# koadman/mauveAligner

Hardware: AMD Instinct MI355X
Metric: aligned Mbp/s (seed+extend+DP) (higher is better)
Workload: dtype u32; 1 GPU; C3: 5 x 5000000 bp synthetic genomes, ~3% divergence, ~50 inversions, seed weight 15, recursive anchoring + gapped DP on; genomes_per_gpu=5, genome_length=5000000, seed_weight=15, parallelism=independent genome sets per GPU (no data-path collective), extend_lcbs=1, max_extension_iters=4

## Files before the change

### mauvealigner_amd/csrc/radix_sort.hip

```cpp
#include "radix_sort.hpp"
#include <algorithm>
#include <cstdlib>

template <typename KeyT>
__global__ void __launch_bounds__(RS_THREADS) rs_hist(const KeyT *__restrict__ keys, uint32_t n, int shift,
                                                      uint32_t *__restrict__ hist, uint32_t nblk)
{
    __shared__ uint32_t h[256];
    h[threadIdx.x] = 0;
    __syncthreads();
    const uint32_t base = blockIdx.x * RS_TILE;
    if (base + RS_TILE <= n) {
        constexpr int KPV = 16 / (int)sizeof(KeyT);
        struct alignas(16) Vec { KeyT k[KPV]; };
        const Vec *src = reinterpret_cast<const Vec *>(keys + base);
#pragma unroll
        for (int i = 0; i < RS_ITEMS / KPV; i++) {
            const Vec q = src[i * RS_THREADS + threadIdx.x];
#pragma unroll
            for (int j = 0; j < KPV; j++) atomicAdd(&h[(uint32_t)(q.k[j] >> shift) & 255u], 1u);
        }
    } else {
#pragma unroll
        for (int i = 0; i < RS_ITEMS; i++) {
// ... 37 lines not shown
    for (uint32_t i0 = lo; i0 < hi; i0 += 512) {
        uint32_t v[8];
#pragma unroll
        for (int q = 0; q < 8; q++) { const uint32_t idx = i0 + q * 64 + lane; v[q] = idx < hi ? row[idx] : 0u; }
#pragma unroll
        for (int q = 0; q < 8; q++) {
            const uint32_t idx = i0 + q * 64 + lane;
            const uint32_t inc = wave_incl_sum_u32(v[q]);
            if (idx < hi) row[idx] = run + inc - v[q];
            run += (uint32_t)__builtin_amdgcn_readlane((int32_t)inc, 63);
        }
    }
    if (threadIdx.x == 0) totals[blockIdx.x] = total;
}

template <typename KeyT, bool RAW = false, typename ValT = uint32_t>
__global__ void __launch_bounds__(RS_THREADS) rs_scatter(const KeyT *__restrict__ keys_in,
                                                         const ValT *__restrict__ vals_in,
                                                         KeyT *__restrict__ keys_out,
                                                         ValT *__restrict__ vals_out, uint32_t n, int shift,
                                                         const uint32_t *__restrict__ hist,
                                                         const uint32_t *__restrict__ totals, uint32_t nblk)
{
    __shared__ KeyT s_keys[RS_TILE];
    __shared__ ValT s_vals[RS_TILE];
    __shared__ uint32_t wcount[RS_WAVES][256];
    __shared__ uint32_t gbase[256];
    __shared__ uint32_t tstart[256];
    __shared__ uint32_t scan[256];

    const int tid = threadIdx.x;
// ... 2 lines not shown

    for (int w = 0; w < RS_WAVES; w++) wcount[w][tid] = 0;
    if (RAW) {
        const uint32_t *row = hist + (size_t)tid * nblk;
        uint32_t tot = 0, before = 0;
        for (uint32_t t = 0; t < nblk; t++) { const uint32_t c = row[t]; tot += c; before += t < blockIdx.x ? c : 0u; }
        uint32_t dummy;
        gbase[tid] = block_excl_scan(tot, &dummy, scan) + before;
    } else {
        uint32_t dummy;
        const uint32_t tot = totals[tid];
        gbase[tid] = block_excl_scan(tot, &dummy, scan) + hist[(size_t)tid * nblk + blockIdx.x];
    }
    __syncthreads();
    if (tile_n == RS_TILE)
        rs_scatter_tile<KeyT, RS_ITEMS, true, ValT>(keys_in, vals_in, keys_out, vals_out, tile_base, tile_n, shift, s_keys, s_vals, wcount, gbase, tstart, scan);
    else
        rs_scatter_tile<KeyT, RS_ITEMS, false, ValT>(keys_in, vals_in, keys_out, vals_out, tile_base, tile_n, shift, s_keys, s_vals, wcount, gbase, tstart, scan);
}

static bool small_sort_on() { static const bool v = [] { const char *e = getenv("MAUVE_SMALL_SORT"); return !(e && e[0] == '0'); }(); return v; }

template <typename KeyT, typename ValT>
int sort_pairs(mauve_ctx *ctx, uint32_t n, int key_bits, KeyT **keys_io, ValT **vals_io, KeyT *keys_alt, ValT *vals_alt, bool have_hist0,
               int timer_id, int shift_lo)
{
    const int k_hist = timer_id >= 0 ? timer_id : MAUVE_K_SORT_HIST, k_scan = timer_id >= 0 ? timer_id : MAUVE_K_SORT_SCAN,
              k_scat = timer_id >= 0 ? timer_id : MAUVE_K_SORT_SCATTER;
    if (small_sort_on() && !have_hist0 && n >= 1 && n <= SS_CAP) {
        HIPCHK(ctx, ctx->hist.ensure(ss_ws_words(n) * sizeof(uint32_t)));
        small_sort<KeyT>(ctx->stream, n, key_bits, shift_lo, keys_io, vals_io, keys_alt, vals_alt, ctx->hist.as<uint32_t>(),
                         [&](bool scatter, auto &&launch) { KernelTimer t(ctx, scatter ? k_scat : k_hist, n); launch(); });
        HIPCHK(ctx, hipGetLastError());
        return MAUVE_OK;
    }
    uint32_t nblk = (n + RS_TILE - 1) / RS_TILE;
    HIPCHK(ctx, ctx->hist.ensure((size_t)nblk * 256 * sizeof(uint32_t)));
    HIPCHK(ctx, ctx->totals.ensure(256 * sizeof(uint32_t)));
    KeyT *kin = *keys_io, *kout = keys_alt; ValT *vin = *vals_io, *vout = vals_alt;
    for (int shift = shift_lo; shift < key_bits; shift += 8) {
        if (!(shift == shift_lo && have_hist0)) { KernelTimer t(ctx, k_hist, n);
          hipLaunchKernelGGL(rs_hist<KeyT>, dim3(nblk), dim3(RS_THREADS), 0, ctx->stream, kin, n, shift,
                             ctx->hist.as<uint32_t>(), nblk); }
        if (nblk <= 64) {
            KernelTimer t(ctx, k_scat, n);
            hipLaunchKernelGGL((rs_scatter<KeyT, true, ValT>), dim3(nblk), dim3(RS_THREADS), 0, ctx->stream, kin, vin, kout, vout, n,
                               shift, ctx->hist.as<uint32_t>(), ctx->totals.as<uint32_t>(), nblk);
            std::swap(kin, kout); std::swap(vin, vout);
            continue;
        }
        { KernelTimer t(ctx, k_scan, n);
          hipLaunchKernelGGL(rs_rowscan, dim3(256), dim3(256), 0, ctx->stream, ctx->hist.as<uint32_t>(), nblk,
                             ctx->totals.as<uint32_t>()); }
        { KernelTimer t(ctx, k_scat, n);
          hipLaunchKernelGGL((rs_scatter<KeyT, false, ValT>), dim3(nblk), dim3(RS_THREADS), 0, ctx->stream, kin, vin, kout, vout, n,
                             shift, ctx->hist.as<uint32_t>(), ctx->totals.as<uint32_t>(), nblk); }
        std::swap(kin, kout); std::swap(vin, vout);
    }
    HIPCHK(ctx, hipGetLastError());
    *keys_io = kin; *vals_io = vin;
    return MAUVE_OK;
}
RS_SORT_PAIRS(uint32_t, uint32_t);
RS_SORT_PAIRS(uint32_t, uint64_t);
RS_SORT_PAIRS(uint64_t, uint32_t);
RS_SORT_PAIRS(uint64_t, uint64_t);

int sort_pairs_u32(mauve_ctx *ctx, uint32_t n, int key_bits, uint32_t **keys_io, uint32_t **vals_io, uint32_t *keys_alt, uint32_t *vals_alt,
                   int timer_id)
{
    return sort_pairs<uint32_t>(ctx, n, key_bits, keys_io, vals_io, keys_alt, vals_alt, false, timer_id);
// ... 30 lines not shown
```

### mauvealigner_amd/csrc/radix_sort.hpp

```cpp
#pragma once
#include "common.hpp"
#include "small_sort.hpp"

constexpr int RS_ITEMS = 16;
constexpr int RS_TILE = RS_THREADS * RS_ITEMS;

template <typename KeyT, typename ValT = uint32_t>
int sort_pairs(mauve_ctx *ctx, uint32_t n, int key_bits, KeyT **keys_io, ValT **vals_io, KeyT *keys_alt, ValT *vals_alt, bool have_hist0,
               int timer_id = -1, int shift_lo = 0);
#define RS_SORT_PAIRS(KeyT, ValT) template int sort_pairs<KeyT, ValT>(mauve_ctx *, uint32_t, int, KeyT **, ValT **, KeyT *, ValT *, bool, int, int)
extern RS_SORT_PAIRS(uint32_t, uint32_t);
extern RS_SORT_PAIRS(uint32_t, uint64_t);
extern RS_SORT_PAIRS(uint64_t, uint32_t);
extern RS_SORT_PAIRS(uint64_t, uint64_t);
```

### mauvealigner_amd/csrc/seed_pass.hip

```cpp
#include "common.hpp"
#include "dev_scan.hpp"
#include "radix_sort.hpp"
#include "seed_dev.hpp"
#include <algorithm>
#include <cstring>
#include <cstdlib>
#include <type_traits>

__device__ __forceinline__ uint32_t seg_of(const uint32_t *__restrict__ segs, uint32_t nseg, uint32_t p)
{
    uint32_t lo = 0, hi = nseg;
    while (hi - lo > 1) { uint32_t mid = (lo + hi) >> 1; if (segs[mid] <= p) lo = mid; else hi = mid; }
    return lo;
}
__device__ __forceinline__ bool window_segment(const uint32_t *__restrict__ seg, uint32_t nseg, int g, uint32_t p, int span, uint32_t *id)
{
    const uint32_t *sg = seg + (size_t)g * (nseg + 1);
    const uint32_t k = *id = seg_of(sg, nseg, p);
    return p + span <= sg[k + 1];
}

template <typename KeyT, bool SEG, typename ValT = uint32_t>
__global__ void __launch_bounds__(256) seed_extract(const uint64_t *__restrict__ packed, GenomeTab tab,
                                                    SeedShape sh, int g, KeyT *__restrict__ keys,
// ... 8 lines not shown
        if (SEG) {
            uint32_t k;
            key = window_segment(seg, nseg, g, p, sh.span, &k) ? (((uint64_t)k << (2 * sh.weight)) | key) : ~0ULL;
        }
        keys[out_base + p] = (KeyT)key;
        vals[out_base + p] = win_make<ValT>(tab.gpos_off[g] + p, m.strand);
    }
}

template <typename KeyT, bool SEG, bool NARROW, typename ValT = uint32_t>
__global__ void __launch_bounds__(256) seed_extract_all(const uint64_t *__restrict__ packed, GenomeTab tab, SeedShape sh,
                                                        KeyT *__restrict__ keys, ValT *__restrict__ vals, uint32_t P,
                                                        const uint32_t *__restrict__ seg, uint32_t nseg,
                                                        uint32_t *__restrict__ hist, uint32_t nblk,
                                                        const uint64_t *__restrict__ vmask, int hist_shift,
                                                        const uint64_t *__restrict__ cmask)
{
    __shared__ uint32_t h[256];
    h[threadIdx.x] = 0;
    __syncthreads();
    const uint32_t base = blockIdx.x * 4096u;
#pragma unroll 2
    for (int i = 0; i < 4; i++) {
        const uint32_t gp0 = base + i * 1024 + threadIdx.x * 4;
        if (gp0 >= P) break;
        const int g0 = genome_of(gp0, tab);
        const bool together = gp0 + 3 < P && gp0 + 3 < tab.gpos_off[g0 + 1];
        uint64_t key[4]; uint32_t sf[4];
        if (together) {
            const uint32_t p0 = gp0 - tab.gpos_off[g0];
            const uint64_t *G = packed + tab.word_off[g0];
            const uint32_t q = p0 >> 5; const int r0 = (p0 & 31) * 2;
            const uint64_t w0 = G[q], w1 = G[q + 1], w2 = G[q + 2], w3 = NARROW ? 0ULL : G[q + 3];
#pragma unroll
// ... 17 lines not shown
        }
        if (SEG || vmask || cmask) {
#pragma unroll
            for (int j = 0; j < 4; j++) {
                const uint32_t gp = gp0 + j;
                if (gp >= P) continue;
                const int g = together ? g0 : genome_of(gp, tab);
                const uint32_t p = gp - tab.gpos_off[g];
                if (SEG) {
                    uint32_t k;
                    key[j] = window_segment(seg, nseg, g, p, sh.span, &k) ? (((uint64_t)k << (2 * sh.weight)) | key[j]) : ~0ULL;
                }
                if ((vmask || cmask) && window_blocked(vmask ? vmask + tab.mask_off[g] : nullptr, cmask ? cmask + tab.mask_off[g] : nullptr, p, sh.span)) key[j] = ~0ULL;
            }
        }
        if (gp0 + 3 < P) {
            if (sizeof(KeyT) == 4) *reinterpret_cast<uint4 *>(keys + gp0) = make_uint4((uint32_t)key[0], (uint32_t)key[1], (uint32_t)key[2], (uint32_t)key[3]);
            else {
                reinterpret_cast<ulonglong2 *>(keys + gp0)[0] = make_ulonglong2(key[0], key[1]);
                reinterpret_cast<ulonglong2 *>(keys + gp0)[1] = make_ulonglong2(key[2], key[3]);
            }
            if constexpr (sizeof(ValT) == 4)
                *reinterpret_cast<uint4 *>(vals + gp0) = make_uint4(gp0 | (sf[0] << 31), (gp0 + 1) | (sf[1] << 31), (gp0 + 2) | (sf[2] << 31), (gp0 + 3) | (sf[3] << 31));
            else {
                reinterpret_cast<ulonglong2 *>(vals + gp0)[0] = make_ulonglong2(win_make<ValT>(gp0, sf[0]), win_make<ValT>(gp0 + 1, sf[1]));
                reinterpret_cast<ulonglong2 *>(vals + gp0)[1] = make_ulonglong2(win_make<ValT>(gp0 + 2, sf[2]), win_make<ValT>(gp0 + 3, sf[3]));
            }
#pragma unroll
            for (int j = 0; j < 4; j++) atomicAdd(&h[(uint32_t)((KeyT)key[j] >> hist_shift) & 255u], 1u);
        } else {
            for (int j = 0; j < 4 && gp0 + j < P; j++) {
                keys[gp0 + j] = (KeyT)key[j]; vals[gp0 + j] = win_make<ValT>(gp0 + j, sf[j]);
                atomicAdd(&h[(uint32_t)((KeyT)key[j] >> hist_shift) & 255u], 1u);
            }
        }
    }
    __syncthreads();
    hist[threadIdx.x * nblk + blockIdx.x] = h[threadIdx.x];
}

__device__ __forceinline__ bool window_valid(uint32_t gp, uint32_t P, const GenomeTab &tab, int span, const uint64_t *__restrict__ vmask,
                                             const uint64_t *__restrict__ cmask)
{
    if (gp >= P) return false;
    const int g = genome_of(gp, tab);
    return !window_blocked(vmask ? vmask + tab.mask_off[g] : nullptr, cmask ? cmask + tab.mask_off[g] : nullptr, gp - tab.gpos_off[g], span);
}

__global__ void __launch_bounds__(256) valid_count(GenomeTab tab, int span, uint32_t P, const uint64_t *__restrict__ vmask,
                                                   uint32_t *__restrict__ tile_cnt, const uint64_t *__restrict__ cmask)
{
    __shared__ uint32_t lds[8];
    const uint32_t first = blockIdx.x * 4096u + threadIdx.x * 16u;
// ... 213 lines not shown
        const uint32_t m = finder_components(mode, once, multi, want_mask);
        if (!(m & gbit[r])) continue;
        mm[r] = m;
        if ((m & (0u - m)) == gbit[r]) skey[slot[r]] = sizeof(ValT) == 4 ? (KeyT)v[r] : (KeyT)win_idx(v[r]);
    }
    __syncthreads();
#pragma unroll
    for (int r = 0; r < HJ_ROWS; r++) {
        if (!mm[r]) continue;
        const uint32_t ap = sizeof(ValT) == 4 ? (uint32_t)skey[slot[r]] & 0x7fffffffu : (uint32_t)skey[slot[r]];
        if (ap >= P) { atomicAdd(&ovf_cnt[1], 1u); continue; }
        const int g = __ffs(gbit[r]) - 1;
        tpos[(size_t)ap * tab.nseq + g] = hit_word(v[r], tab.gpos_off[g]);
        if ((mm[r] & (0u - mm[r])) == gbit[r]) tmask[ap] = mm[r];
    }
}

constexpr int TJ_SLOTS = 16384;
constexpr int TJ_MAX = 9216;
constexpr int TJ_ROWS = TJ_MAX / 1024;
template <bool LOCAL = false>
__global__ void __launch_bounds__(1024) tiny_join(const uint64_t *__restrict__ packed, GenomeTab tab, SeedShape sh, uint32_t P,
                                                  const uint64_t *__restrict__ vmask, const uint64_t *__restrict__ cmask, int mode, uint32_t want_mask,
                                                  uint32_t *__restrict__ tmask, uint32_t *__restrict__ tpos, uint32_t *__restrict__ err_cnt,
                                                  const uint32_t *__restrict__ seg, uint32_t nseg, uint32_t *__restrict__ counters, uint32_t clr_lo, uint32_t clr_hi)
{
    extern __shared__ uint32_t tj_lds[];
    uint32_t *skey = tj_lds, *som = tj_lds + TJ_SLOTS;
    constexpr uint32_t EMPTY = 0xffffffffu;
    const int tid = threadIdx.x;
// ... 533 lines not shown
    tab->gpos_off[gs.nseq] = (uint32_t)tot;
    for (int g = gs.nseq + 1; g <= MAUVE_MAX_SEQ; g++) tab->gpos_off[g] = 0xffffffffu;
    *total_windows = tot;
    return MAUVE_OK;
}

struct FinderPass { uint32_t consider, want; int rule; };

struct SeedPlan {
    bool seg;
    bool hash_path;
    bool tiny;
    bool compact;
    bool has_invalid;
    bool use_summary;
    int segbits;
    int full_bits;
    int low_bits(uint32_t entries) const
    {
        if (!hash_path) return 0;
        int G = 0;
        while (G < full_bits && ((uint64_t)entries >> G) > 512) G += 8;
        if (seg) G = std::max(G, (segbits + 7) / 8 * 8);
        return full_bits - std::min(G, full_bits);
    }
};

static int seed_plan(mauve_ctx *ctx, const SeedShape &sh, const GenomeTab &tab, const SeedRequest &rq, uint32_t n, bool masked, bool seg,
                     int key_type_bits, SeedPlan *pl, std::vector<FinderPass> *passes)
{
    pl->seg = seg;
    pl->hash_path = !rq.hits && rq.mode != MAUVE_MODE_PAIRWISE && !rq.out_keys && !rq.enumerate && rq.only_seq < 0 && !(masked && seg);
    pl->segbits = 0;
    if (seg) while (pl->segbits < 32 && (1ull << pl->segbits) <= (uint64_t)rq.nseg) pl->segbits++;
    if (seg && 2 * sh.weight + pl->segbits > 64) { ctx->err = "recursive anchoring: segment id and mer do not fit 64 bits"; return MAUVE_ERR_LIMIT; }
    pl->full_bits = seg ? 2 * sh.weight + pl->segbits : ((masked && rq.only_seq >= 0) ? key_type_bits : 2 * sh.weight);
    pl->tiny = pl->hash_path && !no_tiny() && n <= (uint32_t)TJ_MAX && tab.nseq <= 16 && 2 * sh.weight + pl->segbits <= 32;
    pl->compact = !rq.hits && !pl->tiny && rq.only_seq < 0 && masked && !seg;
    pl->has_invalid = masked && !pl->compact;
    const int N = tab.nseq;
    if (rq.mode == MAUVE_MODE_PAIRWISE) {
        int pi = 0;
        for (int i = 0; i < N; i++) for (int j = i + 1; j < N; j++, pi++)
            if (!ctx->pair_sums_only || !ctx->shard_on || pi % ctx->shard_world == ctx->shard_rank)
                passes->push_back({(1u << i) | (1u << j), (1u << i) | (1u << j), MAUVE_MODE_MEM});
    } else passes->push_back({0xffffffffu, (uint32_t)rq.mask, rq.mode});
    pl->use_summary = rq.mode == MAUVE_MODE_PAIRWISE && !seg && !rq.hits && (passes->size() > 1 || (ctx->pair_sums_only && ctx->shard_on && !passes->empty()));
    return MAUVE_OK;
}

struct SeedState {
    mauve_ctx *ctx; const GenomeSet &gs; const SeedShape &sh; const GenomeTab &tab; const SeedRequest &rq;
    uint32_t P;
    const uint64_t *packed, *vmask, *cmask;
    SeedPlan pl;
    std::vector<FinderPass> passes;
    uint32_t ns = 0;
    int L = 0;
    uint32_t *tmask = nullptr, *tpos = nullptr;
    uint32_t cand_cap = 0;
    uint32_t cand_total = 0;
    bool records_on_host = false;
    double trace_t0 = 0;
};
template <typename KeyT, typename ValT>
struct SeedPass : SeedState {
    KeyT *keys = nullptr; ValT *vals = nullptr;
    bool have_hist0 = false;
    SeedPass(const SeedState &s) : SeedState(s) {}
};

template <typename KeyT, typename ValT>
static int ensure_sort_buffers(mauve_ctx *ctx, uint32_t n)
{
    HIPCHK(ctx, ctx->keysA.ensure((size_t)n * sizeof(KeyT)));
    HIPCHK(ctx, ctx->keysB.ensure((size_t)n * sizeof(KeyT)));
    HIPCHK(ctx, ctx->valsA.ensure((size_t)n * sizeof(ValT)));
    HIPCHK(ctx, ctx->valsB.ensure((size_t)n * sizeof(ValT)));
    return MAUVE_OK;
}

template <typename F>
static void launch_narrow_or_not(const SeedShape &sh, F &&launch)
{
    if (seed_narrow(sh)) launch(std::true_type{});
    else launch(std::false_type{});
}

template <typename KeyT, bool SEG, typename ValT>
static int extract_all(mauve_ctx *ctx, const GenomeSet &gs, const SeedShape &sh, const GenomeTab &tab, uint32_t n, const uint32_t *seg, uint32_t nseg,
                       int hshift, KeyT *keys, ValT *vals)
{
    const uint32_t nblk = (n + RS_TILE - 1) / RS_TILE;
    HIPCHK(ctx, ctx->hist.ensure((size_t)nblk * 256 * sizeof(uint32_t)));
    const uint64_t *packed = gs.buf->as<uint64_t>();
    const uint64_t *vmask = gs.vmask ? gs.vmask->as<uint64_t>() : nullptr;
    const uint64_t *cmask = gs.cmask ? gs.cmask->as<uint64_t>() : nullptr;
    KernelTimer t(ctx, MAUVE_K_EXTRACT, n);
    launch_narrow_or_not(sh, [&](auto narrow) {
        hipLaunchKernelGGL((seed_extract_all<KeyT, SEG, decltype(narrow)::value, ValT>), dim3(nblk), dim3(256), 0, ctx->stream, packed, tab, sh, keys,
                           vals, n, seg, nseg, ctx->hist.as<uint32_t>(), nblk, vmask, hshift, cmask);
    });
    return MAUVE_OK;
}

template <typename KeyT, bool SEG, typename ValT>
static int extract(SeedPass<KeyT, ValT> &ps)
{
    mauve_ctx *ctx = ps.ctx; const SeedRequest &rq = ps.rq; const uint32_t n = ps.P;
    if (int rc = ensure_sort_buffers<KeyT, ValT>(ctx, n)) return rc;
    HIPCHK(ctx, ctx->counters.ensure(64));
    KeyT *keys = ps.keys = ctx->keysA.as<KeyT>(); ValT *vals = ps.vals = ctx->valsA.as<ValT>();
    if (rq.hits) ps.ns = 1;
    else if (ps.pl.tiny) ps.ns = n;
    else if (ps.pl.compact) {
        const uint32_t nblk = (n + 4095) / 4096;
// ... 1 lines not shown
        uint32_t *tile_cnt = ctx->hist.as<uint32_t>();
        {
            KernelTimer t(ctx, MAUVE_K_EXTRACT, n);
            hipLaunchKernelGGL(valid_count, dim3(nblk), dim3(256), 0, ctx->stream, ps.tab, ps.sh.span, n, ps.vmask, tile_cnt, ps.cmask);
            hipLaunchKernelGGL(tile_scan, dim3(1), dim3(256), 0, ctx->stream, tile_cnt, nblk, ctx->counters.as<uint32_t>());
            launch_narrow_or_not(ps.sh, [&](auto narrow) {
                hipLaunchKernelGGL((seed_extract_compact<KeyT, decltype(narrow)::value, ValT>), dim3(nblk), dim3(256), 0, ctx->stream, ps.packed, ps.tab, ps.sh,
                                   keys, vals, n, ps.vmask, tile_cnt, ps.cmask);
            });
        }
        HIPCHK(ctx, hipGetLastError());
        const uint32_t *cw;
        if (int rc = seed_counters(ctx, 16, &cw)) return rc;
        ps.ns = cw[0];
    } else if (rq.only_seq < 0) {
        if (int rc = extract_all<KeyT, SEG, ValT>(ctx, ps.gs, ps.sh, ps.tab, n, rq.seg, rq.nseg, ps.pl.low_bits(n), keys, vals)) return rc;
        ps.ns = n; ps.have_hist0 = true;
    } else {
        const int g = rq.only_seq;
        uint32_t nw = ps.tab.nwin[g];
        if (nw) {
            uint32_t blocks = std::min<uint32_t>((nw + 255) / 256, 256 * 16);
            KernelTimer t(ctx, MAUVE_K_EXTRACT, nw);
            hipLaunchKernelGGL((seed_extract<KeyT, SEG, ValT>), dim3(blocks), dim3(256), 0, ctx->stream, ps.packed, ps.tab, ps.sh, g, keys,
                               vals, 0u, rq.seg, rq.nseg);
            ps.ns = nw;
        }
    }
    HIPCHK(ctx, hipGetLastError());
    seed_trace(ctx, "extract", ps.trace_t0);
    return MAUVE_OK;
}
// ... 49 lines not shown
    out_keys->resize(sorted_n);
    for (uint32_t i = 0; i < sorted_n; i++) (*out_keys)[i] = (uint64_t)hk[i];
    if (WIDEV) {
        const uint32_t g0 = ps.tab.gpos_off[ps.rq.only_seq];
        for (uint32_t i = 0; i < sorted_n; i++) (*out_vals)[i] = ((uint32_t)hv[i] - g0) | ((uint32_t)((uint64_t)hv[i] >> 63) << 31);
    }
    return MAUVE_OK;
}

static bool cand_overflow(SeedState &st, uint32_t nc)
{
    if (nc > st.cand_cap) st.ctx->err = "seed pass: " + std::to_string(nc) + " candidates for a list of " + std::to_string(st.cand_cap);
    return nc > st.cand_cap;
}

template <bool SEG>
static int launch_runs(SeedState &st)
{
    mauve_ctx *ctx = st.ctx; const uint32_t P = st.P;
    { KernelTimer t(ctx, MAUVE_K_RUNS, P);
      hipLaunchKernelGGL((mum_runs<SEG>), dim3((P + RUNS_TILE - 1) / RUNS_TILE), dim3(256), 0, ctx->stream, st.tab,
                         st.sh.span, st.tmask, st.tpos, P, st.rq.extend ? 0 : 1, ctx->cand.as<uint32_t>(), ctx->counters.as<uint32_t>(), st.rq.seg,
                         st.rq.nseg, st.cand_cap, 0u); }
    HIPCHK(ctx, hipGetLastError());
    return MAUVE_OK;
}

template <bool SEG, bool WIDEV>
static int launch_extend(SeedState &st, uint32_t blocks, uint32_t ncand, int32_t *o_len, int32_t *o_start, const uint32_t *ncand_dev = nullptr,
                         uint32_t *counters_out = nullptr)
{
    mauve_ctx *ctx = st.ctx;
    KernelTimer t(ctx, MAUVE_K_EXTEND, ncand);
    hipLaunchKernelGGL((mum_extend<SEG, WIDEV>), dim3(blocks), dim3(256), 0, ctx->stream, st.packed, st.tab, st.sh, st.tmask, st.tpos, st.P,
                       ctx->cand.as<uint32_t>(), ncand, st.rq.extend, o_len, o_start, st.rq.seg, st.rq.nseg, st.vmask, st.cmask, ncand_dev, counters_out);
    HIPCHK(ctx, hipGetLastError());
#ifdef MAUVE_EXT_STATS
    if (seed_trace_on()) {
// ... 80 lines not shown
    return MAUVE_OK;
}

static_assert(TJ_MAX / 2 + 1 <= 8192, "a tiny pass's candidate list: extension launched for its capacity");
template <bool SEG, bool WIDEV>
static int tiny_pass(SeedState &st, const FinderPass &fp)
{
    mauve_ctx *ctx = st.ctx; const uint32_t P = st.P, cand_cap = st.cand_cap; const int N = st.tab.nseq;
    static const bool tj_attr = hipFuncSetAttribute(reinterpret_cast<const void *>(tiny_join<WIDEV>), hipFuncAttributeMaxDynamicSharedMemorySize, TJ_SLOTS * 8) == hipSuccess;
    if (!tj_attr) { ctx->err = "tiny_join: cannot reserve its LDS"; return MAUVE_ERR_HIP; }
    { KernelTimer t(ctx, MAUVE_K_JOIN, P);
      hipLaunchKernelGGL(tiny_join<WIDEV>, dim3(1), dim3(1024), TJ_SLOTS * 8, ctx->stream, st.packed, st.tab, st.sh, P, st.vmask, st.cmask, fp.rule, fp.want, st.tmask, st.tpos,
                         ctx->counters.as<uint32_t>() + 9, SEG ? st.rq.seg : (const uint32_t *)nullptr, st.rq.nseg, ctx->counters.as<uint32_t>(), 0u, P); }
    HIPCHK(ctx, hipGetLastError());
    seed_trace(ctx, "join", st.trace_t0);
    if (int rc = launch_runs<SEG>(st)) return rc;
    if (ctx->shadow) { std::function<void()> f; f.swap(ctx->shadow); f(); }
    const size_t lbytes = ((size_t)cand_cap * 4 + 63) & ~(size_t)63, sbytes = (size_t)cand_cap * 4 * N;
    HIPCHK(ctx, ctx->pin_seed.ensure(64 + lbytes + sbytes));
    char *pin = ctx->pin_seed.as<char>();
    const bool host_out = cand_cap < canon_device_min();
    if (!host_out) { HIPCHK(ctx, ctx->mlen.ensure((size_t)cand_cap * 4 + 4)); HIPCHK(ctx, ctx->mstart.ensure((size_t)cand_cap * 4 * N + 4)); }
    int32_t *o_len = host_out ? reinterpret_cast<int32_t *>(pin + 64) : ctx->mlen.as<int32_t>();
    int32_t *o_st = host_out ? reinterpret_cast<int32_t *>(pin + 64 + lbytes) : ctx->mstart.as<int32_t>();
    if (int rc = launch_extend<SEG, WIDEV>(st, std::min<uint32_t>((cand_cap + 3) / 4, 512), cand_cap, o_len, o_st, ctx->counters.as<uint32_t>() + 1,
                                           reinterpret_cast<uint32_t *>(pin))) return rc;
    if (!host_out) {
        HIPCHK(ctx, hipMemcpyAsync(pin + 64, ctx->mlen.p, (size_t)cand_cap * 4, hipMemcpyDeviceToHost, ctx->stream));
        HIPCHK(ctx, hipMemcpyAsync(pin + 64 + lbytes, ctx->mstart.p, sbytes, hipMemcpyDeviceToHost, ctx->stream));
    }
    HIPCHK(ctx, hipStreamSynchronize(ctx->stream));
// ... 35 lines not shown
    }
    if (tot_sl) {
        HIPCHK(ctx, ctx->join_bound.ensure((2 * nsl + 1) * 4));
        HIPCHK(ctx, ctx->pin_seed.ensure(64 + (2 * nsl + 1) * 4));
        uint32_t *hp = reinterpret_cast<uint32_t *>(ctx->pin_seed.as<char>() + 64);
        memcpy(hp, sl_lo.data(), nsl * 4); memcpy(hp + nsl, sl_pre.data(), (nsl + 1) * 4);
        HIPCHK(ctx, hipMemcpyAsync(ctx->join_bound.p, hp, (2 * nsl + 1) * 4, hipMemcpyHostToDevice, ctx->stream));
        KernelTimer t(ctx, MAUVE_K_JOIN, (uint32_t)tot_sl);
        hipLaunchKernelGGL((mum_join_slices<KeyT, SEG, ValT>), dim3((uint32_t)((tot_sl + 255) / 256)), dim3(256), 0, ctx->stream, (const KeyT *)keys, (const ValT *)vals,
                           ctx->join_bound.as<uint32_t>(), ctx->join_bound.as<uint32_t>() + nsl, (uint32_t)nsl, ps.tab, fp.rule, fp.want,
                           fp.consider, ps.tmask, ps.tpos, (int)ps.pl.has_invalid);
        HIPCHK(ctx, hipStreamSynchronize(ctx->stream));
    }
    HIPCHK(ctx, hipGetLastError());
    HIPCHK(ctx, hipMemsetAsync(ctx->counters.p, 0, 64, ctx->stream));
    if (int rc = launch_runs<SEG>(ps)) return rc;
    const uint32_t *cw;
    if (int rc = seed_counters(ctx, 16, &cw)) return rc;
    *nc = cw[1];
    if (seed_trace_on()) fprintf(stderr, "[trace]   join_hash handed back %u range(s)\n", novf);
    return MAUVE_OK;
}

template <typename KeyT, bool SEG, typename ValT>
static int finder_pass(SeedPass<KeyT, ValT> &ps, const FinderPass &fp)
{
    constexpr bool WIDEV = sizeof(ValT) == 8;
    mauve_ctx *ctx = ps.ctx; const uint32_t P = ps.P, ns = ps.ns; const int N = ps.tab.nseq;
    const HostHits *hh = ps.rq.hits;
    HIPCHK(ctx, hipMemsetAsync(ps.tmask, 0, (size_t)P * 4, ctx->stream));
    HIPCHK(ctx, hipMemsetAsync(ctx->counters.p, 0, 64, ctx->stream));
    if (hh) {
        HIPCHK(ctx, ctx->run_sum.ensure((size_t)hh->n * (N + 1) * 4 + 64));
        HIPCHK(ctx, hipMemcpyAsync(ctx->run_sum.p, hh->rec, (size_t)hh->n * (N + 1) * 4, hipMemcpyHostToDevice, ctx->stream));
        if (hh->n) hipLaunchKernelGGL(hits_scatter<WIDEV>, dim3((hh->n + 255) / 256), dim3(256), 0, ctx->stream, ctx->run_sum.as<uint32_t>(), hh->n, N, P, ps.tmask, ps.tpos, ps.tab);
        HIPCHK(ctx, hipStreamSynchronize(ctx->stream));
    } else if (ps.pl.hash_path) {
        const uint32_t nchunk = (ns + HJ_T - 1) / HJ_T;
        HIPCHK(ctx, ctx->join_ovf.ensure((2 + 2 * (size_t)HJ_OVF_CAP) * 4));
        KernelTimer t(ctx, MAUVE_K_JOIN, ns);
        HIPCHK(ctx, ctx->join_bound.ensure(((size_t)nchunk + 2) * 4));
        hipLaunchKernelGGL((join_bounds<KeyT>), dim3((nchunk + 1 + 3) / 4), dim3(256), 0, ctx->stream, ps.keys, ns, ps.L, nchunk,
                           ctx->join_bound.as<uint32_t>());
#define JH_LAUNCH(W) hipLaunchKernelGGL((join_hash<KeyT, W, ValT>), dim3(nchunk), dim3(256), 0, ctx->stream, ps.keys, ps.vals, ns, \
                                           ctx->join_bound.as<uint32_t>(), ps.tab, fp.rule, fp.want, ps.tmask, ps.tpos, ctx->counters.as<uint32_t>() + 8, ctx->join_ovf.as<uint32_t>(), P)
        if (N > 16) JH_LAUNCH(true);
        else JH_LAUNCH(false);
#undef JH_LAUNCH
    } else
    { KernelTimer t(ctx, MAUVE_K_JOIN, ns);
      hipLaunchKernelGGL((mum_join<KeyT, SEG, ValT>), dim3((ns + 255) / 256), dim3(256), 0, ctx->stream, ps.keys, ps.vals, ns, ps.tab, fp.rule,
                         fp.want, fp.consider, ps.tmask, ps.tpos, P, (int)ps.pl.has_invalid); }
    HIPCHK(ctx, hipGetLastError());
    seed_trace(ctx, "join", ps.trace_t0);
    if (int rc = launch_runs<SEG>(ps)) return rc;
    if (ctx->shadow) { std::function<void()> f; f.swap(ctx->shadow); f(); }
    const uint32_t *cw;
    if (int rc = seed_counters(ctx, 48, &cw)) return rc;
    uint32_t nc = cw[1];
    const uint32_t novf = ps.pl.hash_path ? cw[8] : 0u;
    if (ps.pl.hash_path && cw[9]) { ctx->err = "join_hash: anchor out of range (internal error)"; return MAUVE_ERR_HIP; }
    if (novf) if (int rc = join_overflow_slices<KeyT, SEG, ValT>(ps, fp, novf, &nc)) return rc;
    if (cand_overflow(ps, nc)) return MAUVE_ERR_LIMIT;
    seed_trace(ctx, "runs", ps.trace_t0);
    if (seed_trace_on()) fprintf(stderr, "[trace]   %u candidates of %u windows\n", nc, P);
    if (nc == 0) return MAUVE_OK;
    constexpr int EXT_BLOCKS_PER_CU = 12;
    return extend_candidates<SEG, WIDEV>(ps, nc, (uint32_t)(ctx->cus * EXT_BLOCKS_PER_CU));
}

template <typename KeyT, bool SEG, typename ValT>
static int seedpass_stages(const SeedState &st0)
{
    constexpr bool WIDEV = sizeof(ValT) == 8;
    SeedPass<KeyT, ValT> ps(st0);
    mauve_ctx *ctx = ps.ctx; const SeedRequest &rq = ps.rq; const uint32_t P = ps.P; const int N = ps.tab.nseq;
    if (seed_trace_on()) fprintf(stderr, "[trace] seed pass: %u windows, %d-bit keys, %s window index (%d-bit values)\n", P, (int)sizeof(KeyT) * 8,
                                  WIDEV ? "wide" : "narrow", (int)sizeof(ValT) * 8);
    if (int rc = seed_plan(ctx, ps.sh, ps.tab, rq, P, ps.vmask || ps.cmask, SEG, (int)sizeof(KeyT) * 8, &ps.pl, &ps.passes)) return rc;
    if (int rc = extract<KeyT, SEG, ValT>(ps)) return rc;
    if (ps.ns == 0) { if (rq.n_matches) *rq.n_matches = 0; return MAUVE_OK; }
    ps.L = ps.pl.low_bits(ps.ns);
    if (!rq.hits && !ps.pl.tiny)
        if (int rc = sort_pairs<KeyT, ValT>(ctx, ps.ns, ps.pl.full_bits, &ps.keys, &ps.vals, ctx->keysB.as<KeyT>(), ctx->valsB.as<ValT>(), ps.have_hist0, -1, ps.L)) return rc;
    seed_trace(ctx, "sort", ps.trace_t0);
    if (rq.enumerate) return export_enumerator(ps);
    if (rq.out_keys) return export_sorted_list(ps);

    HIPCHK(ctx, ctx->posmask.ensure((size_t)P * 4));
    HIPCHK(ctx, ctx->hit_pos.ensure((size_t)P * 4 * N));
    ps.tmask = ctx->posmask.as<uint32_t>(); ps.tpos = ctx->hit_pos.as<uint32_t>();
    ps.cand_cap = P / 2 + 1;
    HIPCHK(ctx, ctx->cand.ensure((size_t)ps.cand_cap * 4));
    if (list_cap_env()) ps.cand_cap = std::min(ps.cand_cap, list_cap_env());
    ctx->sdh.hl.clear(); ctx->sdh.hs.clear();
    if (ps.pl.tiny) {
        if (int rc = tiny_pass<SEG, WIDEV>(ps, ps.passes[0])) return rc;
    } else if (ps.pl.use_summary) {
        if (int rc = pairwise_passes(ps)) return rc;
// ... 194 lines not shown
```

### mauvealigner_amd/csrc/small_sort.hpp

```cpp
#pragma once
#include <hip/hip_runtime.h>
#include <cstdint>

constexpr int RS_THREADS = 256;
constexpr int RS_WAVES = RS_THREADS / 64;

__device__ __forceinline__ uint32_t block_excl_scan(uint32_t v, uint32_t *total, uint32_t *lds )
{
    const int lane = threadIdx.x & 63, wave = threadIdx.x >> 6;
    uint32_t inc = v;
#pragma unroll
    for (int o = 1; o < 64; o <<= 1) { uint32_t t = __shfl_up(inc, o); if (lane >= o) inc += t; }
    if (lane == 63) lds[wave] = inc;
    __syncthreads();
    uint32_t wbase = 0, tot = 0;
#pragma unroll
    for (int w = 0; w < 4; w++) { uint32_t c = lds[w]; if (w < wave) wbase += c; tot += c; }
    __syncthreads();
    *total = tot;
    return wbase + inc - v;
}

template <typename KeyT, int ITEMS, bool FULL, typename ValT = uint32_t>
__device__ __forceinline__ void rs_scatter_tile(const KeyT *__restrict__ keys_in, const ValT *__restrict__ vals_in,
                                                KeyT *__restrict__ keys_out, ValT *__restrict__ vals_out,
                                                uint32_t tile_base, uint32_t tile_n, int shift, KeyT *s_keys, ValT *s_vals,
                                                uint32_t (*wcount)[256], const uint32_t *gbase, uint32_t *tstart, uint32_t *scan,
                                                uint32_t *__restrict__ hnext = nullptr, int tile_log2 = 0, int hbits = 0)
{
    const int tid = threadIdx.x, lane = tid & 63, wave = tid >> 6;
    KeyT k[ITEMS]; ValT v[ITEMS]; uint32_t rank[ITEMS];
    const uint32_t wbase = wave * (64 * ITEMS);
#pragma unroll
    for (int i = 0; i < ITEMS; i++) {
        const uint32_t li = wbase + i * 64 + lane;
        const bool ok = FULL || li < tile_n;
        k[i] = ok ? keys_in[tile_base + li] : (KeyT)0;
        v[i] = ok ? vals_in[tile_base + li] : (ValT)0;
    }
    uint32_t *wc = wcount[wave];
#pragma unroll
    for (int i = 0; i < ITEMS; i++) {
        const uint32_t li = wbase + i * 64 + lane;
        const bool ok = FULL || li < tile_n;
        const uint32_t d = (uint32_t)(k[i] >> shift) & 255u;
        uint32_t plo, phi;
        if (FULL) { plo = 0xffffffffu; phi = 0xffffffffu; }
        else { const uint64_t a = __ballot(ok); plo = (uint32_t)a; phi = (uint32_t)(a >> 32); }
#pragma unroll
        for (int b = 0; b < 8; b++) {
            const uint64_t m = FULL ? __ballot((d >> b) & 1) : __ballot(ok && ((d >> b) & 1));
            const uint32_t sb = (uint32_t)((int32_t)(d << (31 - b)) >> 31);
            plo &= ~((uint32_t)m ^ sb); phi &= ~((uint32_t)(m >> 32) ^ sb);
// ... 174 lines not shown
```

Before: 10110 Mbp/s.

## Pack strand bits into a bitmap and synthesize sort values in first scatter

Seed extraction no longer writes a full per-window value array. It now writes a compact bitmap of strand flags per tile, and the first radix scatter pass reconstructs each value from the element index plus the bitmap bit. The finder pass replaces the full-array memset of the mask with a custom clear kernel limited to the window range the pass anchors on, and restricts mum_runs to that range. This cuts global memory writes and reads of the value stream and the clear cost, but adds template variants and a dependency on the first pass being tiled.

```diff
diff --git a/mauvealigner_amd/csrc/radix_sort.hip b/mauvealigner_amd/csrc/radix_sort.hip
--- a/mauvealigner_amd/csrc/radix_sort.hip
+++ b/mauvealigner_amd/csrc/radix_sort.hip
@@ -75,7 +75,7 @@
     if (threadIdx.x == 0) totals[blockIdx.x] = total;
 }
 
-template <typename KeyT, bool RAW = false, typename ValT = uint32_t>
+template <typename KeyT, bool RAW = false, typename ValT = uint32_t, bool IOTA = false>
 __global__ void __launch_bounds__(RS_THREADS) rs_scatter(const KeyT *__restrict__ keys_in,
                                                          const ValT *__restrict__ vals_in,
                                                          KeyT *__restrict__ keys_out,
@@ -108,19 +108,22 @@
     }
     __syncthreads();
     if (tile_n == RS_TILE)
-        rs_scatter_tile<KeyT, RS_ITEMS, true, ValT>(keys_in, vals_in, keys_out, vals_out, tile_base, tile_n, shift, s_keys, s_vals, wcount, gbase, tstart, scan);
+        rs_scatter_tile<KeyT, RS_ITEMS, true, ValT, IOTA>(keys_in, vals_in, keys_out, vals_out, tile_base, tile_n, shift, s_keys, s_vals, wcount, gbase, tstart, scan,
+                                                          nullptr, 0, 0, reinterpret_cast<const uint64_t *>(vals_in));
     else
-        rs_scatter_tile<KeyT, RS_ITEMS, false, ValT>(keys_in, vals_in, keys_out, vals_out, tile_base, tile_n, shift, s_keys, s_vals, wcount, gbase, tstart, scan);
+        rs_scatter_tile<KeyT, RS_ITEMS, false, ValT, IOTA>(keys_in, vals_in, keys_out, vals_out, tile_base, tile_n, shift, s_keys, s_vals, wcount, gbase, tstart, scan,
+                                                           nullptr, 0, 0, reinterpret_cast<const uint64_t *>(vals_in));
 }
 
 static bool small_sort_on() { static const bool v = [] { const char *e = getenv("MAUVE_SMALL_SORT"); return !(e && e[0] == '0'); }(); return v; }
 
 template <typename KeyT, typename ValT>
 int sort_pairs(mauve_ctx *ctx, uint32_t n, int key_bits, KeyT **keys_io, ValT **vals_io, KeyT *keys_alt, ValT *vals_alt, bool have_hist0,
-               int timer_id, int shift_lo)
+               int timer_id, int shift_lo, bool iota)
 {
     const int k_hist = timer_id >= 0 ? timer_id : MAUVE_K_SORT_HIST, k_scan = timer_id >= 0 ? timer_id : MAUVE_K_SORT_SCAN,
               k_scat = timer_id >= 0 ? timer_id : MAUVE_K_SORT_SCATTER;
+    if (iota && !(have_hist0 && shift_lo < key_bits)) { ctx->err = "sort_pairs: values from the strand bitmap need a first tiled pass"; return MAUVE_ERR_ARG; }
     if (small_sort_on() && !have_hist0 && n >= 1 && n <= SS_CAP) {
         HIPCHK(ctx, ctx->hist.ensure(ss_ws_words(n) * sizeof(uint32_t)));
         small_sort<KeyT>(ctx->stream, n, key_bits, shift_lo, keys_io, vals_io, keys_alt, vals_alt, ctx->hist.as<uint32_t>(),
@@ -136,10 +139,11 @@
         if (!(shift == shift_lo && have_hist0)) { KernelTimer t(ctx, k_hist, n);
           hipLaunchKernelGGL(rs_hist<KeyT>, dim3(nblk), dim3(RS_THREADS), 0, ctx->stream, kin, n, shift,
                              ctx->hist.as<uint32_t>(), nblk); }
+        const bool first_iota = iota && shift == shift_lo;
         if (nblk <= 64) {
             KernelTimer t(ctx, k_scat, n);
-            hipLaunchKernelGGL((rs_scatter<KeyT, true, ValT>), dim3(nblk), dim3(RS_THREADS), 0, ctx->stream, kin, vin, kout, vout, n,
-                               shift, ctx->hist.as<uint32_t>(), ctx->totals.as<uint32_t>(), nblk);
+            hipLaunchKernelGGL((first_iota ? rs_scatter<KeyT, true, ValT, true> : rs_scatter<KeyT, true, ValT, false>), dim3(nblk), dim3(RS_THREADS), 0, ctx->stream,
+                               kin, vin, kout, vout, n, shift, ctx->hist.as<uint32_t>(), ctx->totals.as<uint32_t>(), nblk);
             std::swap(kin, kout); std::swap(vin, vout);
             continue;
         }
@@ -147,8 +151,8 @@
           hipLaunchKernelGGL(rs_rowscan, dim3(256), dim3(256), 0, ctx->stream, ctx->hist.as<uint32_t>(), nblk,
                              ctx->totals.as<uint32_t>()); }
         { KernelTimer t(ctx, k_scat, n);
-          hipLaunchKernelGGL((rs_scatter<KeyT, false, ValT>), dim3(nblk), dim3(RS_THREADS), 0, ctx->stream, kin, vin, kout, vout, n,
-                             shift, ctx->hist.as<uint32_t>(), ctx->totals.as<uint32_t>(), nblk); }
+          hipLaunchKernelGGL((first_iota ? rs_scatter<KeyT, false, ValT, true> : rs_scatter<KeyT, false, ValT, false>), dim3(nblk), dim3(RS_THREADS), 0, ctx->stream,
+                             kin, vin, kout, vout, n, shift, ctx->hist.as<uint32_t>(), ctx->totals.as<uint32_t>(), nblk); }
         std::swap(kin, kout); std::swap(vin, vout);
     }
     HIPCHK(ctx, hipGetLastError());
diff --git a/mauvealigner_amd/csrc/radix_sort.hpp b/mauvealigner_amd/csrc/radix_sort.hpp
--- a/mauvealigner_amd/csrc/radix_sort.hpp
+++ b/mauvealigner_amd/csrc/radix_sort.hpp
@@ -7,8 +7,8 @@
 
 template <typename KeyT, typename ValT = uint32_t>
 int sort_pairs(mauve_ctx *ctx, uint32_t n, int key_bits, KeyT **keys_io, ValT **vals_io, KeyT *keys_alt, ValT *vals_alt, bool have_hist0,
-               int timer_id = -1, int shift_lo = 0);
-#define RS_SORT_PAIRS(KeyT, ValT) template int sort_pairs<KeyT, ValT>(mauve_ctx *, uint32_t, int, KeyT **, ValT **, KeyT *, ValT *, bool, int, int)
+               int timer_id = -1, int shift_lo = 0, bool iota = false);
+#define RS_SORT_PAIRS(KeyT, ValT) template int sort_pairs<KeyT, ValT>(mauve_ctx *, uint32_t, int, KeyT **, ValT **, KeyT *, ValT *, bool, int, int, bool)
 extern RS_SORT_PAIRS(uint32_t, uint32_t);
 extern RS_SORT_PAIRS(uint32_t, uint64_t);
 extern RS_SORT_PAIRS(uint64_t, uint32_t);
diff --git a/mauvealigner_amd/csrc/seed_pass.hip b/mauvealigner_amd/csrc/seed_pass.hip
--- a/mauvealigner_amd/csrc/seed_pass.hip
+++ b/mauvealigner_amd/csrc/seed_pass.hip
@@ -46,10 +46,12 @@
                                                         const uint32_t *__restrict__ seg, uint32_t nseg,
                                                         uint32_t *__restrict__ hist, uint32_t nblk,
                                                         const uint64_t *__restrict__ vmask, int hist_shift,
-                                                        const uint64_t *__restrict__ cmask)
+                                                        const uint64_t *__restrict__ cmask, uint32_t *__restrict__ sbits)
 {
     __shared__ uint32_t h[256];
+    __shared__ uint32_t sb[4096 / 32];
     h[threadIdx.x] = 0;
+    if (threadIdx.x < 4096 / 32) sb[threadIdx.x] = 0;
     __syncthreads();
     const uint32_t base = blockIdx.x * 4096u;
 #pragma unroll 2
@@ -97,13 +99,15 @@
                 if ((vmask || cmask) && window_blocked(vmask ? vmask + tab.mask_off[g] : nullptr, cmask ? cmask + tab.mask_off[g] : nullptr, p, sh.span)) key[j] = ~0ULL;
             }
         }
+        if (sbits) atomicOr(&sb[(gp0 - base) >> 5], (sf[0] | sf[1] << 1 | sf[2] << 2 | sf[3] << 3) << ((gp0 - base) & 31u));
         if (gp0 + 3 < P) {
             if (sizeof(KeyT) == 4) *reinterpret_cast<uint4 *>(keys + gp0) = make_uint4((uint32_t)key[0], (uint32_t)key[1], (uint32_t)key[2], (uint32_t)key[3]);
             else {
                 reinterpret_cast<ulonglong2 *>(keys + gp0)[0] = make_ulonglong2(key[0], key[1]);
                 reinterpret_cast<ulonglong2 *>(keys + gp0)[1] = make_ulonglong2(key[2], key[3]);
             }
-            if constexpr (sizeof(ValT) == 4)
+            if (sbits) {}
+            else if constexpr (sizeof(ValT) == 4)
                 *reinterpret_cast<uint4 *>(vals + gp0) = make_uint4(gp0 | (sf[0] << 31), (gp0 + 1) | (sf[1] << 31), (gp0 + 2) | (sf[2] << 31), (gp0 + 3) | (sf[3] << 31));
             else {
                 reinterpret_cast<ulonglong2 *>(vals + gp0)[0] = make_ulonglong2(win_make<ValT>(gp0, sf[0]), win_make<ValT>(gp0 + 1, sf[1]));
@@ -113,13 +117,15 @@
             for (int j = 0; j < 4; j++) atomicAdd(&h[(uint32_t)((KeyT)key[j] >> hist_shift) & 255u], 1u);
         } else {
             for (int j = 0; j < 4 && gp0 + j < P; j++) {
-                keys[gp0 + j] = (KeyT)key[j]; vals[gp0 + j] = win_make<ValT>(gp0 + j, sf[j]);
+                keys[gp0 + j] = (KeyT)key[j];
+                if (!sbits) vals[gp0 + j] = win_make<ValT>(gp0 + j, sf[j]);
                 atomicAdd(&h[(uint32_t)((KeyT)key[j] >> hist_shift) & 255u], 1u);
             }
         }
     }
     __syncthreads();
     hist[threadIdx.x * nblk + blockIdx.x] = h[threadIdx.x];
+    if (sbits && threadIdx.x < 4096 / 32) sbits[(size_t)blockIdx.x * (4096 / 32) + threadIdx.x] = sb[threadIdx.x];
 }
 
 __device__ __forceinline__ bool window_valid(uint32_t gp, uint32_t P, const GenomeTab &tab, int span, const uint64_t *__restrict__ vmask,
@@ -363,6 +369,17 @@
         tpos[(size_t)ap * tab.nseq + g] = hit_word(v[r], tab.gpos_off[g]);
         if ((mm[r] & (0u - mm[r])) == gbit[r]) tmask[ap] = mm[r];
     }
+}
+
+__global__ void __launch_bounds__(256) pass_clear(uint32_t *__restrict__ t, uint32_t n, uint32_t *__restrict__ counters)
+{
+    if (blockIdx.x == 0 && threadIdx.x < 16) counters[threadIdx.x] = 0;
+    const uint32_t head = (uint32_t)((reinterpret_cast<uintptr_t>(t) >> 2) & 3u);
+    const uint64_t w = ((uint64_t)blockIdx.x * 256u + threadIdx.x) * 4u;
+    if (w >= (uint64_t)head + n) return;
+    uint32_t *line = t - head + w;
+    if (w >= head && w + 4 <= (uint64_t)head + n) *reinterpret_cast<uint4 *>(line) = make_uint4(0u, 0u, 0u, 0u);
+    else for (uint32_t j = 0; j < 4; j++) if (w + j >= head && w + j < (uint64_t)head + n) line[j] = 0;
 }
 
 constexpr int TJ_SLOTS = 16384;
@@ -926,6 +943,7 @@
     bool compact;
     bool has_invalid;
     bool use_summary;
+    bool strand_bitmap;
     int segbits;
     int full_bits;
     int low_bits(uint32_t entries) const
@@ -950,6 +968,7 @@
     pl->tiny = pl->hash_path && !no_tiny() && n <= (uint32_t)TJ_MAX && tab.nseq <= 16 && 2 * sh.weight + pl->segbits <= 32;
     pl->compact = !rq.hits && !pl->tiny && rq.only_seq < 0 && masked && !seg;
     pl->has_invalid = masked && !pl->compact;
+    pl->strand_bitmap = !rq.hits && !pl->tiny && !pl->compact && rq.only_seq < 0 && pl->low_bits(n) < pl->full_bits;
     const int N = tab.nseq;
     if (rq.mode == MAUVE_MODE_PAIRWISE) {
         int pi = 0;
@@ -979,6 +998,7 @@
 struct SeedPass : SeedState {
     KeyT *keys = nullptr; ValT *vals = nullptr;
     bool have_hist0 = false;
+    bool iota = false;
     SeedPass(const SeedState &s) : SeedState(s) {}
 };
 
@@ -1001,7 +1021,7 @@
 
 template <typename KeyT, bool SEG, typename ValT>
 static int extract_all(mauve_ctx *ctx, const GenomeSet &gs, const SeedShape &sh, const GenomeTab &tab, uint32_t n, const uint32_t *seg, uint32_t nseg,
-                       int hshift, KeyT *keys, ValT *vals)
+                       int hshift, KeyT *keys, ValT *vals, bool bitmap = false)
 {
     const uint32_t nblk = (n + RS_TILE - 1) / RS_TILE;
     HIPCHK(ctx, ctx->hist.ensure((size_t)nblk * 256 * sizeof(uint32_t)));
@@ -1011,7 +1031,7 @@
     KernelTimer t(ctx, MAUVE_K_EXTRACT, n);
     launch_narrow_or_not(sh, [&](auto narrow) {
         hipLaunchKernelGGL((seed_extract_all<KeyT, SEG, decltype(narrow)::value, ValT>), dim3(nblk), dim3(256), 0, ctx->stream, packed, tab, sh, keys,
-                           vals, n, seg, nseg, ctx->hist.as<uint32_t>(), nblk, vmask, hshift, cmask);
+                           vals, n, seg, nseg, ctx->hist.as<uint32_t>(), nblk, vmask, hshift, cmask, bitmap ? reinterpret_cast<uint32_t *>(vals) : nullptr);
     });
     return MAUVE_OK;
 }
@@ -1043,8 +1063,10 @@
         if (int rc = seed_counters(ctx, 16, &cw)) return rc;
         ps.ns = cw[0];
     } else if (rq.only_seq < 0) {
-        if (int rc = extract_all<KeyT, SEG, ValT>(ctx, ps.gs, ps.sh, ps.tab, n, rq.seg, rq.nseg, ps.pl.low_bits(n), keys, vals)) return rc;
-        ps.ns = n; ps.have_hist0 = true;
+        if (ps.pl.strand_bitmap) HIPCHK(ctx, ctx->valsA.ensure(std::max((size_t)n * sizeof(ValT), (size_t)((n + RS_TILE - 1) / RS_TILE) * (RS_TILE / 8))));
+        vals = ps.vals = ctx->valsA.as<ValT>();
+        if (int rc = extract_all<KeyT, SEG, ValT>(ctx, ps.gs, ps.sh, ps.tab, n, rq.seg, rq.nseg, ps.pl.low_bits(n), keys, vals, ps.pl.strand_bitmap)) return rc;
+        ps.ns = n; ps.have_hist0 = true; ps.iota = ps.pl.strand_bitmap;
     } else {
         const int g = rq.only_seq;
         uint32_t nw = ps.tab.nwin[g];
@@ -1124,14 +1146,31 @@
     return nc > st.cand_cap;
 }
 
+struct WinRange { uint32_t lo, hi; };
+static WinRange anchor_range(const GenomeTab &tab, uint32_t P, const FinderPass &fp, bool host_hits)
+{
+    const int N = tab.nseq;
+    const uint32_t in_set = N >= 32 ? 0xffffffffu : (1u << N) - 1u;
+    WinRange r{0u, P};
+    if (host_hits) return r;
+    if (fp.want) {
+        const int g = __builtin_ctz(fp.want);
+        if (g < N) r = {tab.gpos_off[g], tab.gpos_off[g + 1]};
+    } else if (const uint32_t c = fp.consider & in_set)
+        r = {tab.gpos_off[__builtin_ctz(c)], tab.gpos_off[31 - __builtin_clz(c)]};
+    r.hi = std::min(r.hi, P);
+    if (r.lo >= r.hi) r = {0u, P};
+    return r;
+}
+
 template <bool SEG>
-static int launch_runs(SeedState &st)
-{
-    mauve_ctx *ctx = st.ctx; const uint32_t P = st.P;
-    { KernelTimer t(ctx, MAUVE_K_RUNS, P);
-      hipLaunchKernelGGL((mum_runs<SEG>), dim3((P + RUNS_TILE - 1) / RUNS_TILE), dim3(256), 0, ctx->stream, st.tab,
-                         st.sh.span, st.tmask, st.tpos, P, st.rq.extend ? 0 : 1, ctx->cand.as<uint32_t>(), ctx->counters.as<uint32_t>(), st.rq.seg,
-                         st.rq.nseg, st.cand_cap, 0u); }
+static int launch_runs(SeedState &st, WinRange r)
+{
+    mauve_ctx *ctx = st.ctx;
+    { KernelTimer t(ctx, MAUVE_K_RUNS, r.hi - r.lo);
+      hipLaunchKernelGGL((mum_runs<SEG>), dim3((r.hi - r.lo + RUNS_TILE - 1) / RUNS_TILE), dim3(256), 0, ctx->stream, st.tab,
+                         st.sh.span, st.tmask, st.tpos, r.hi, st.rq.extend ? 0 : 1, ctx->cand.as<uint32_t>(), ctx->counters.as<uint32_t>(), st.rq.seg,
+                         st.rq.nseg, st.cand_cap, r.lo); }
     HIPCHK(ctx, hipGetLastError());
     return MAUVE_OK;
 }
@@ -1242,7 +1281,7 @@
                          ctx->counters.as<uint32_t>() + 9, SEG ? st.rq.seg : (const uint32_t *)nullptr, st.rq.nseg, ctx->counters.as<uint32_t>(), 0u, P); }
     HIPCHK(ctx, hipGetLastError());
     seed_trace(ctx, "join", st.trace_t0);
-    if (int rc = launch_runs<SEG>(st)) return rc;
+    if (int rc = launch_runs<SEG>(st, WinRange{0u, P})) return rc;
     if (ctx->shadow) { std::function<void()> f; f.swap(ctx->shadow); f(); }
     const size_t lbytes = ((size_t)cand_cap * 4 + 63) & ~(size_t)63, sbytes = (size_t)cand_cap * 4 * N;
     HIPCHK(ctx, ctx->pin_seed.ensure(64 + lbytes + sbytes));
@@ -1308,7 +1347,7 @@
     }
     HIPCHK(ctx, hipGetLastError());
     HIPCHK(ctx, hipMemsetAsync(ctx->counters.p, 0, 64, ctx->stream));
-    if (int rc = launch_runs<SEG>(ps)) return rc;
+    if (int rc = launch_runs<SEG>(ps, anchor_range(ps.tab, ps.P, fp, false))) return rc;
     const uint32_t *cw;
     if (int rc = seed_counters(ctx, 16, &cw)) return rc;
     *nc = cw[1];
@@ -1322,8 +1361,9 @@
     constexpr bool WIDEV = sizeof(ValT) == 8;
     mauve_ctx *ctx = ps.ctx; const uint32_t P = ps.P, ns = ps.ns; const int N = ps.tab.nseq;
     const HostHits *hh = ps.rq.hits;
-    HIPCHK(ctx, hipMemsetAsync(ps.tmask, 0, (size_t)P * 4, ctx->stream));
-    HIPCHK(ctx, hipMemsetAsync(ctx->counters.p, 0, 64, ctx->stream));
+    const WinRange ar = anchor_range(ps.tab, P, fp, hh != nullptr);
+    const uint32_t clr_lo = ar.lo >= RUNS_HALO ? ar.lo - RUNS_HALO : 0u;
+    hipLaunchKernelGGL(pass_clear, dim3((ar.hi - clr_lo + 3) / 1024 + 1), dim3(256), 0, ctx->stream, ps.tmask + clr_lo, ar.hi - clr_lo, ctx->counters.as<uint32_t>());
     if (hh) {
         HIPCHK(ctx, ctx->run_sum.ensure((size_t)hh->n * (N + 1) * 4 + 64));
         HIPCHK(ctx, hipMemcpyAsync(ctx->run_sum.p, hh->rec, (size_t)hh->n * (N + 1) * 4, hipMemcpyHostToDevice, ctx->stream));
@@ -1347,7 +1387,7 @@
                          fp.want, fp.consider, ps.tmask, ps.tpos, P, (int)ps.pl.has_invalid); }
     HIPCHK(ctx, hipGetLastError());
     seed_trace(ctx, "join", ps.trace_t0);
-    if (int rc = launch_runs<SEG>(ps)) return rc;
+    if (int rc = launch_runs<SEG>(ps, ar)) return rc;
     if (ctx->shadow) { std::function<void()> f; f.swap(ctx->shadow); f(); }
     const uint32_t *cw;
     if (int rc = seed_counters(ctx, 48, &cw)) return rc;
@@ -1376,7 +1416,7 @@
     if (ps.ns == 0) { if (rq.n_matches) *rq.n_matches = 0; return MAUVE_OK; }
     ps.L = ps.pl.low_bits(ps.ns);
     if (!rq.hits && !ps.pl.tiny)
-        if (int rc = sort_pairs<KeyT, ValT>(ctx, ps.ns, ps.pl.full_bits, &ps.keys, &ps.vals, ctx->keysB.as<KeyT>(), ctx->valsB.as<ValT>(), ps.have_hist0, -1, ps.L)) return rc;
+        if (int rc = sort_pairs<KeyT, ValT>(ctx, ps.ns, ps.pl.full_bits, &ps.keys, &ps.vals, ctx->keysB.as<KeyT>(), ctx->valsB.as<ValT>(), ps.have_hist0, -1, ps.L, ps.iota)) return rc;
     seed_trace(ctx, "sort", ps.trace_t0);
     if (rq.enumerate) return export_enumerator(ps);
     if (rq.out_keys) return export_sorted_list(ps);
diff --git a/mauvealigner_amd/csrc/small_sort.hpp b/mauvealigner_amd/csrc/small_sort.hpp
--- a/mauvealigner_amd/csrc/small_sort.hpp
+++ b/mauvealigner_amd/csrc/small_sort.hpp
@@ -21,22 +21,33 @@
     return wbase + inc - v;
 }
 
-template <typename KeyT, int ITEMS, bool FULL, typename ValT = uint32_t>
+template <typename KeyT, int ITEMS, bool FULL, typename ValT = uint32_t, bool IOTA = false>
 __device__ __forceinline__ void rs_scatter_tile(const KeyT *__restrict__ keys_in, const ValT *__restrict__ vals_in,
                                                 KeyT *__restrict__ keys_out, ValT *__restrict__ vals_out,
                                                 uint32_t tile_base, uint32_t tile_n, int shift, KeyT *s_keys, ValT *s_vals,
                                                 uint32_t (*wcount)[256], const uint32_t *gbase, uint32_t *tstart, uint32_t *scan,
-                                                uint32_t *__restrict__ hnext = nullptr, int tile_log2 = 0, int hbits = 0)
+                                                uint32_t *__restrict__ hnext = nullptr, int tile_log2 = 0, int hbits = 0,
+                                                const uint64_t *__restrict__ sbits = nullptr)
 {
     const int tid = threadIdx.x, lane = tid & 63, wave = tid >> 6;
     KeyT k[ITEMS]; ValT v[ITEMS]; uint32_t rank[ITEMS];
     const uint32_t wbase = wave * (64 * ITEMS);
+    uint32_t sb_lo = 0, sb_hi = 0;
+    if (IOTA) {
+        const uint64_t w = lane < ITEMS ? sbits[(size_t)((tile_base + wbase) >> 6) + (uint32_t)lane] : 0ULL;
+        sb_lo = (uint32_t)w; sb_hi = (uint32_t)(w >> 32);
+    }
 #pragma unroll
     for (int i = 0; i < ITEMS; i++) {
         const uint32_t li = wbase + i * 64 + lane;
         const bool ok = FULL || li < tile_n;
         k[i] = ok ? keys_in[tile_base + li] : (KeyT)0;
-        v[i] = ok ? vals_in[tile_base + li] : (ValT)0;
+        if (IOTA) {
+            const uint32_t lo = (uint32_t)__builtin_amdgcn_readlane((int32_t)sb_lo, i), hi = (uint32_t)__builtin_amdgcn_readlane((int32_t)sb_hi, i);
+            const uint32_t half = lane < 32 ? lo : hi;
+            v[i] = ok ? (ValT)(tile_base + li) | ((ValT)((half >> (lane & 31)) & 1u) << (8 * sizeof(ValT) - 1)) : (ValT)0;
+        } else
+            v[i] = ok ? vals_in[tile_base + li] : (ValT)0;
     }
     uint32_t *wc = wcount[wave];
 #pragma unroll
```

After: 10320 Mbp/s, median of 6. 2.1% higher.
